# emreatilgan/P-Companion

Hardware: AMD Instinct MI355X
Metric: triplets/sec (Product2Vec pretrain step: gather+fwd+bwd+Adam) + P-Companion joint step under `joint` (higher is better)
Workload: dtype f32

## Files before the change

include/pcompanion_hip.h:

```cpp
#ifndef PCOMPANION_HIP_H
#define PCOMPANION_HIP_H

#include <stddef.h>
#include <stdint.h>

#ifdef __cplusplus
extern "C" {
#endif

#define PC_OK 0
#define PC_EINVAL (-1)
#define PC_ESHAPE (-2)
#define PC_EWORKSPACE (-3)
#define PC_EBATCHNORM (-4)
#define PC_ECOMM (-5)

#define PC_D 128
#define PC_H 256
#define PC_HEADS 4
#define PC_L 64
#define PC_MAX_SEG 4
#define PC_BN_SYNC_DOUBLES (PC_MAX_SEG * 2 * 256 + PC_MAX_SEG)

#define PC_ABI_VERSION 8
int pc_abi_version(void);
enum { PC_OPT_SIDE_QUEUE = 1, PC_OPT_SORTED_TABLE_GRADIENTS = 2, PC_OPT_BN_FINALIZE_SIDE = 3, PC_OPT_FUSED_LOSS = 4,
       PC_OPT_FUSED_OUT_CHAIN = 5, PC_OPT_BN_FINALIZE_RIDES = 6 };
int pc_set_option(int option, int value);
int pc_get_option(int option, int* value);
int pc_release_device_state(void);
enum {
    PC_FLAG_EXP_NO_MFMA = 1, PC_FLAG_EXP_NO_SPLIT = 2, PC_FLAG_EXP_NO_LDSREAD = 4, PC_FLAG_EXP_NO_DMA = 8,
    PC_FLAG_EXP_NO_SLAB = 16, PC_FLAG_EXP_STAGGER = 32, PC_FLAG_EXP_DMA_L2 = 64, PC_FLAG_NT_TIMING = 128,
    PC_FLAG_JOINT_TIMING = 256, PC_FLAG_CHAIN_TIMING = 512, PC_FLAG_EXP_NO_BARRIER = 1024, PC_FLAG_EXP_NO_VMWAIT = 2048
};
unsigned pc_build_flags(void);

typedef struct {
    float p;
    uint64_t seed, offset;
} pc_dropout;

typedef struct {
    float *w0, *b0, *gamma, *beta, *w3, *b3, *w5, *b5;
    float *in_proj_w, *in_proj_b, *out_proj_w, *out_proj_b;
    float *running_mean, *running_var;
    int64_t *num_batches_tracked;
    pc_dropout dropout;
    int dim;
} pc_p2v_tensors;

typedef struct {
    int nseg;
    int start[PC_MAX_SEG + 1];
    int count[PC_MAX_SEG];
    int weighted_row;
    float weight;
    const float *row_weight;
    int row_weight_start, row_weight_rows;
} pc_segments;
// ... 577 lines not shown
```

p_companion_amd/_lib.py:

```python
import ctypes
import os

_HERE = os.path.dirname(os.path.abspath(__file__))
LIB_PATH = os.path.join(_HERE, "libpcompanion_hip.so")
if os.environ.get("PC_DEV_LIB"):
    import sys as _sys
    LIB_PATH = os.path.abspath(os.environ["PC_DEV_LIB"])
    print(f"[p_companion_amd] PC_DEV_LIB: loading {LIB_PATH} instead of the in-tree library (developer A/B run)", file=_sys.stderr, flush=True)

c_f32p = ctypes.c_void_p
c_i32p = ctypes.c_void_p
PC_MAX_SEG = 4
D, H, HEADS, L = 128, 256, 4, 64

_ERR = {-1: "PC_EINVAL (null pointer / bad size)", -2: "PC_ESHAPE (unsupported dimension/alignment)",
        -3: "PC_EWORKSPACE (workspace too small)",
        -4: "PC_EBATCHNORM (a BatchNorm call group of one row in training mode)",
        -5: "PC_ECOMM (RCCL could not be loaded, or a communicator call failed)"}


class HipKernelError(RuntimeError):
    pass


# ... 20 lines not shown
class AttnSaved(ctypes.Structure):
    _fields_ = [(n, ctypes.c_void_p) for n in ("q", "qt", "probs", "c", "sp", "ctx")]


class JointTensors(ctypes.Structure):
    _fields_ = [(n, ctypes.c_void_p) for n in (
        "product_table", "enc_w", "enc_b", "dec_w", "dec_b", "typ_w", "typ_b", "itm_w", "itm_b",
        "query_types", "comp_types")] + [("dropout", Dropout)]


class JointSaved(ctypes.Structure):
    _fields_ = [(n, ctypes.c_void_p) for n in ("h", "c", "pi", "tp")]


_vp, _i, _sz, _f, _d, _u64, _i64 = (ctypes.c_void_p, ctypes.c_int, ctypes.c_size_t, ctypes.c_float,
                                    ctypes.c_double, ctypes.c_uint64, ctypes.c_int64)
_P = ctypes.POINTER

class AdamFused(ctypes.Structure):
    _fields_ = [("param", ctypes.c_void_p), ("grad", ctypes.c_void_p), ("exp_avg", ctypes.c_void_p), ("exp_avg_sq", ctypes.c_void_p),
                ("n", ctypes.c_size_t), ("step_count", ctypes.c_void_p), ("t", ctypes.c_int64),
                ("lr", ctypes.c_double), ("beta1", ctypes.c_double), ("beta2", ctypes.c_double), ("eps", ctypes.c_double)]


class RowWhere(ctypes.Structure):
    _fields_ = [(n, ctypes.c_void_p) for n in ("value", "lo", "hi", "flags", "need", "deny")]


PC_OPT_SIDE_QUEUE = 1
PC_OPT_FUSED_OUT_CHAIN = 5
PC_OPT_FUSED_LOSS = 4
PC_OPT_BN_FINALIZE_SIDE = 3
PC_OPT_BN_FINALIZE_RIDES = 6
PC_OPT_SORTED_TABLE_GRADIENTS = 2

SIGNATURES = {
    "pc_abi_version": (_i, []),
    "pc_build_flags": (ctypes.c_uint, []),
    "pc_set_option": (_i, [_i, _i]),
    "pc_get_option": (_i, [_i, ctypes.POINTER(ctypes.c_int)]),
    "pc_release_device_state": (_i, []),
    "pc_p2v_ffn_workspace_bytes": (_sz, [_i]),
    "pc_p2v_ffn_forward_train": (_i, [_P(P2VTensors), _vp, _vp, _i, _P(Segments), _i, _vp, _P(FfnSaved), _vp, _sz, _vp]),
    "pc_p2v_ffn_forward_eval": (_i, [_P(P2VTensors), _vp, _vp, _i, _vp, _vp, _sz, _vp]),
    "pc_p2v_ffn_backward": (_i, [_P(P2VTensors), _P(P2VTensors), _vp, _vp, _i, _P(Segments), _vp, _P(FfnSaved),
                                 _vp, _i, _vp, _sz, _vp]),
    "pc_p2v_attention_workspace_bytes": (_sz, [_i, _i]),
    "pc_p2v_attention_workspace_bytes_dim": (_sz, [_i, _i, _i]),
    "pc_p2v_attention_forward": (_i, [_P(P2VTensors), _vp, _vp, _i, _i, _vp, _P(AttnSaved), _vp, _sz, _vp]),
    "pc_p2v_attention_backward": (_i, [_P(P2VTensors), _P(P2VTensors), _vp, _vp, _i, _i, _vp, _P(AttnSaved), _vp,
                                       _vp, _i, _vp, _sz, _vp]),
    "pc_p2v_attention_forward_masked": (_i, [_P(P2VTensors), _vp, _vp, _vp, _i, _i, _vp, _P(AttnSaved), _vp, _sz, _vp]),
    "pc_p2v_attention_backward_masked": (_i, [_P(P2VTensors), _P(P2VTensors), _vp, _vp, _vp, _i, _i, _vp, _P(AttnSaved), _vp,
                                              _vp, _i, _vp, _sz, _vp]),
    "pc_p2v_train_step_compact_masked": (_i, [_P(P2VTensors), _P(P2VTensors), _vp, _vp, _vp, _vp, _vp, _i, _vp, _i, _i, _i, _f,
                                              _vp, _vp, _vp, _vp, _vp, _vp, _sz, _vp]),
    "pc_p2v_train_step_unique_masked": (_i, [_P(P2VTensors), _P(P2VTensors), _vp, _vp, _vp, _vp, _vp, _vp, _vp, _i, _i, _vp, _vp,
                                             _vp, _i, _i, _i, _f, _vp, _vp, _vp, _vp, _vp, _vp, _sz, _P(AdamFused), _vp]),
    "pc_p2v_export_workspace_bytes": (_sz, [_i, _i]),
    "pc_p2v_export_embeddings": (_i, [_P(P2VTensors), _vp, _i64, _vp, _vp, _vp, _vp, _i, _vp, _sz, _vp]),
    "pc_p2v_triplet_loss": (_i, [_vp, _vp, _vp, _i, _i, _f, _vp, _vp, _vp, _vp, _vp, _vp, _vp]),
    "pc_p2v_triplet_loss_dim": (_i, [_vp, _vp, _vp, _i, _i, _i, _f, _vp, _vp, _vp, _vp, _vp, _vp, _vp]),
    "pc_adam_step": (_i, [_vp, _vp, _vp, _vp, _sz, _vp, _vp, _d, _d, _d, _d, _vp]),
    "pc_adam_step_at": (_i, [_vp, _vp, _vp, _vp, _sz, _vp, _i64, _d, _d, _d, _d, _vp]),
    "pc_p2v_train_step_workspace_bytes": (_sz, [_i, _i, _i]),
    "pc_p2v_train_step_workspace_bytes_dim": (_sz, [_i, _i, _i, _i]),
# ... 214 lines not shown
```

p_companion_amd/csrc/common.h:

```cpp
#pragma once
#include <hip/hip_runtime.h>
#include <stdint.h>
#include "../../include/pcompanion_hip.h"

typedef float f32x16 __attribute__((ext_vector_type(16)));
typedef float f32x4 __attribute__((ext_vector_type(4)));

#define PC_WAVE 64

#define PC_HIP_TRY(expr)                          \
    do {                                          \
        hipError_t _e = (expr);                   \
        if (_e != hipSuccess) return (int)_e;     \
    } while (0)

#define PC_TRY(expr)                 \
    do {                             \
        int _r = (expr);             \
        if (_r != 0) return _r;      \
    } while (0)

extern thread_local int pc_tls_launch_err;
#define PC_LAUNCH(...)                                                           \
    do {                                                                         \
// ... 44 lines not shown
    for (int i = 0; i < PC_MAX_SEG; i++) {
        si.tile0[i] = t;
        int n = si.start[i + 1] - si.start[i];
        t += (n + tile_rows - 1) / tile_rows;
    }
    si.tile0[PC_MAX_SEG] = t;
    return si;
}

static inline int seg_valid(const pc_segments* s, int rows) {
    if (!s) return 1;
    if (s->nseg < 1 || s->nseg > PC_MAX_SEG || s->start[0] != 0 || s->start[s->nseg] != rows) return 0;
    for (int i = 0; i < s->nseg; i++)
        if (s->start[i + 1] < s->start[i] || s->count[i] < 0) return 0;
    if (s->weighted_row >= rows || (s->weighted_row >= 0 && s->weight < 0.f)) return 0;
    if (s->row_weight && (s->row_weight_start < 0 || s->row_weight_rows < 0 || s->row_weight_start + s->row_weight_rows > rows))
        return 0;
    return 1;
}

#ifdef __HIPCC__
__device__ __forceinline__ int seg_of_row(const SegInfo& si, int r) {
    int s = 0;
#pragma unroll
    for (int i = 1; i < PC_MAX_SEG; i++) s += (i < si.nseg && r >= si.start[i]) ? 1 : 0;
    return s;
}

__device__ __forceinline__ float row_multiplicity(const SegInfo& si, int r) {
#ifdef PC_EXP_NO_ROWMULT
    return 1.f;
#endif
    if (si.roww && (unsigned)(r - si.w0) < (unsigned)si.wn) return si.roww[r - si.w0];
    return r == si.wrow ? si.wmult : 1.f;
}

__device__ __forceinline__ int seg_of_tile(const SegInfo& si, int t) {
    int s = 0;
#pragma unroll
    for (int i = 1; i < PC_MAX_SEG; i++) s += (i < si.nseg && t >= si.tile0[i]) ? 1 : 0;
    return s;
}

__device__ __forceinline__ float fast_tanh(float x) {
    const float e = __builtin_amdgcn_exp2f(x * 2.8853900817779268f);
    return 1.0f - 2.0f * __builtin_amdgcn_rcpf(e + 1.0f);
}

__device__ __forceinline__ float wave_sum(float v) {
#pragma unroll
    for (int o = 32; o >= 1; o >>= 1) v += __shfl_xor(v, o, 64);
    return v;
}

__device__ __forceinline__ float group16_sum(float v) {
#pragma unroll
    for (int o = 8; o >= 1; o >>= 1) v += __shfl_xor(v, o, 64);
    return v;
}

__device__ __forceinline__ f32x16 mfma32(float a, float b, f32x16 c) {
    return __builtin_amdgcn_mfma_f32_32x32x2f32(a, b, c, 0, 0, 0);
}

typedef __bf16 bf16x8 __attribute__((ext_vector_type(8)));
struct Split3 { bf16x8 p0, p1, p2; };
// ... 364 lines not shown
int scatter_add_slab_blocks(int table_rows, int rows, int width);
int launch_scatter_add_slabs(const int32_t* idx, int rows, int width, int table_rows, const float* src, float* slabs,
                             hipStream_t st);

struct WsCarver {
    char* base; size_t total;
    explicit WsCarver(void* b) : base(static_cast<char*>(b)), total(0) {}
    void* bytes(size_t n) {
        void* p = base ? base + total : nullptr;
        total += (n + 255) & ~(size_t)255;
        return p;
    }
    float* floats(size_t n) { return static_cast<float*>(bytes(n * sizeof(float))); }
};

static inline void joint_fields(const pc_joint_tensors* t, float* (&out)[10]) {
    float* const f[10] = {t->itm_w, t->itm_b, t->typ_w, t->typ_b, t->dec_w, t->dec_b, t->enc_w, t->enc_b, t->comp_types, t->query_types};
    for (int i = 0; i < 10; i++) out[i] = f[i];
}
static inline bool joint_tensors_ok(const pc_joint_tensors* t, bool need_table) {
    if (!t || (need_table && !t->product_table)) return false;
    float* f[10];
    joint_fields(t, f);
    for (float* x : f)
        if (!x) return false;
    return true;
}

int pc_opt_sorted_tables();
int pc_opt_bn_finalize_side();
int pc_opt_bn_finalize_rides();
int pc_opt_fused_loss();
int pc_opt_fused_out_chain();
int triplet_loss_launch(const float* a, const float* p, const float* n, int batch, int k_neg, int dim, float margin,
                        float* loss, float* d_pos, float* d_neg, float* da, float* dp, float* dn, void* stream, int with_mean);
int launch_dropout(const float* x, size_t n, const pc_dropout& d, unsigned stream_id, float* y, hipStream_t st);
int launch_transpose(const float* in, int rows, int cols, float* out, hipStream_t st);
struct FfnCall {
    const pc_p2v_tensors *p = nullptr, *g = nullptr;
    const float* table = nullptr;
    const int32_t* idx = nullptr;
    int rows = 0;
    const pc_segments* seg = nullptr;
    const pc_ffn_saved* sv = nullptr;
    void* ws = nullptr; size_t ws_bytes = 0; void* stream = nullptr;
    double* local_sums = nullptr; const double* global_sums = nullptr;
    int update_running = 0; float* y = nullptr;
    const TransposeBatch* ride = nullptr;
    const float* dy = nullptr; float* dx = nullptr;
    int with_dx = 0, transposed = 0;
    int accumulate = 0;
    TnDefer* defer = nullptr;
};
int ffn_forward_part1(const FfnCall& c);
int ffn_forward_part2(const FfnCall& c);
int ffn_backward_part1(const FfnCall& c);
int ffn_backward_part2(const FfnCall& c);
int ffn_transposes(const pc_p2v_tensors* p, void* ws, int rows, int with_dx, TransposeBatch* tb);
int attention_transposes(const pc_p2v_tensors* p, void* ws, int B, int N, int key_rows, TransposeBatch* tb, float* zero_bk);
struct AttnCall {
    const pc_p2v_tensors* p = nullptr;
    const float *query = nullptr, *keys = nullptr;
    int B = 0, N = 0, key_rows = 0;
    const int32_t* slot_row = nullptr;
    const pc_attn_saved* sv = nullptr;
    void* ws = nullptr; size_t ws_bytes = 0; void* stream = nullptr;
// ... 29 lines not shown
```

p_companion_amd/csrc/gemm_tn.hip:

```cpp
#include <atomic>
#include <mutex>
#include <type_traits>
#include "common.h"
#include "bn_finalize.h"
#include "lds_dma.h"

#define TM 128
#define TK 32

__device__ __forceinline__ void tn_small_body(const TnArgs& a, int tiles_i, int nsplit, int rows_per_split, int bid) {
    __shared__ __attribute__((aligned(16))) float smem[2][2][TK * TM];

    const int tid = threadIdx.x, lane = tid & 63, w = tid >> 6, wo = w >> 1, wi = w & 1;
    const int split = bid % nsplit;
    const int tile = bid / nsplit;
    const int o0 = (tile / tiles_i) * TM, i0 = (tile % tiles_i) * TM;
    const int r_begin = split * rows_per_split;
    const int r_end = min(a.R, r_begin + rows_per_split);

    const int lrow = tid >> 5, lcol = (tid & 31) * 4;
    const bool zcol_ok = o0 + lcol < a.No, acol_ok = i0 + lcol < a.Ni;

    float4 rz[4], ra[4];
    float4 dbacc = make_float4(0.f, 0.f, 0.f, 0.f);
    int zseg = -1;
    float4 zmu, zis, zsc, zc1, zc2;
    auto gload = [&](int r0) {
#pragma unroll
        for (int p = 0; p < 4; p++) {
            const int r = r0 + lrow + 8 * p;
            const bool rv = r < r_end;
            if (a.z_onehot) {
                const int t = rv ? a.z_onehot[r] : -1, c = o0 + lcol;
                rz[p] = make_float4(t == c ? 1.f : 0.f, t == c + 1 ? 1.f : 0.f, t == c + 2 ? 1.f : 0.f, t == c + 3 ? 1.f : 0.f);
            } else {
                rz[p] = (rv && zcol_ok) ? *reinterpret_cast<const float4*>(a.Z + (size_t)r * a.ldz + o0 + lcol)
                                        : make_float4(0.f, 0.f, 0.f, 0.f);
            }
            if (a.zaux && rv && zcol_ok) {
                const int s = seg_of_row(a.seg, r);
                if (s != zseg) {
                    const size_t o = (size_t)s * a.No + o0 + lcol;
                    zmu = *reinterpret_cast<const float4*>(a.z_mean + o);
                    zis = *reinterpret_cast<const float4*>(a.z_invstd + o);
                    zsc = *reinterpret_cast<const float4*>(a.z_scale + o);
                    zc1 = *reinterpret_cast<const float4*>(a.z_c1 + o);
                    zc2 = *reinterpret_cast<const float4*>(a.z_c2 + o);
                    zseg = s;
                }
                const float4 h = *reinterpret_cast<const float4*>(a.zaux + (size_t)r * a.ldzaux + o0 + lcol);
                const float zm = row_multiplicity(a.seg, r);
                rz[p].x = zsc.x * (rz[p].x - zm * (zc1.x + (h.x - zmu.x) * zis.x * zc2.x));
                rz[p].y = zsc.y * (rz[p].y - zm * (zc1.y + (h.y - zmu.y) * zis.y * zc2.y));
                rz[p].z = zsc.z * (rz[p].z - zm * (zc1.z + (h.z - zmu.z) * zis.z * zc2.z));
                rz[p].w = zsc.w * (rz[p].w - zm * (zc1.w + (h.w - zmu.w) * zis.w * zc2.w));
            }
            int src = r;
            bool av = rv && acol_ok;
            if (av && a.gather) { src = a.gather[r]; av = src >= 0; }
            ra[p] = av ? *reinterpret_cast<const float4*>(a.A + (size_t)src * a.lda + i0 + lcol)
                       : make_float4(0.f, 0.f, 0.f, 0.f);
            if (a.prologue == NT_PRO_BNTANH && rv && acol_ok) {
                const int s = seg_of_row(a.seg, r);
                const float4 sc = *reinterpret_cast<const float4*>(a.pscale + (size_t)s * a.Ni + i0 + lcol);
                const float4 sh = *reinterpret_cast<const float4*>(a.pshift + (size_t)s * a.Ni + i0 + lcol);
                ra[p].x = fast_tanh(ra[p].x * sc.x + sh.x);
                ra[p].y = fast_tanh(ra[p].y * sc.y + sh.y);
                ra[p].z = fast_tanh(ra[p].z * sc.z + sh.z);
                ra[p].w = fast_tanh(ra[p].w * sc.w + sh.w);
            }
            dbacc.x += rz[p].x; dbacc.y += rz[p].y; dbacc.z += rz[p].z; dbacc.w += rz[p].w;
        }
    };
    auto lstore = [&](int buf) {
#pragma unroll
        for (int p = 0; p < 4; p++) {
            *reinterpret_cast<float4*>(&smem[buf][0][(lrow + 8 * p) * TM + lcol]) = rz[p];
            *reinterpret_cast<float4*>(&smem[buf][1][(lrow + 8 * p) * TM + lcol]) = ra[p];
        }
    };

    f32x16 acc[2][2];
#pragma unroll
    for (int i = 0; i < 2; i++)
#pragma unroll
        for (int j = 0; j < 2; j++)
#pragma unroll
            for (int r = 0; r < 16; r++) acc[i][j][r] = 0.f;
// ... 36 lines not shown
            for (int reg = 0; reg < 16; reg++) {
                const int o = o0 + wo * 64 + mt * 32 + (reg & 3) + 8 * (reg >> 2) + 4 * (lane >> 5);
                if (o < a.No && i < a.Ni) slab[(size_t)o * a.Ni + i] = acc[mt][nt][reg];
            }
        }
    if (a.db && i0 == 0) {
        float* red = &smem[0][0][0];
        *reinterpret_cast<float4*>(&red[lrow * TM + lcol]) = dbacc;
        __syncthreads();
        if (tid < TM && o0 + tid < a.No) {
            float s = 0.f;
#pragma unroll
            for (int g = 0; g < 8; g++) s += red[g * TM + tid];
            slab[(size_t)a.No * a.Ni + o0 + tid] = s;
        }
    }
}

__global__ __launch_bounds__(256, 2) void gemm_tn_kernel(TnArgs a, int tiles_i, int nsplit, int rows_per_split) {
    tn_small_body(a, tiles_i, nsplit, rows_per_split, blockIdx.x);
}

__global__ __launch_bounds__(256, 2) void gemm_tn_group_kernel(TnGroup g) {
    const int b = blockIdx.x;
    int j = 0;
#pragma unroll
    for (int i = 1; i < PC_TN_GROUP; i++) j += (i < g.n && b >= g.block0[i]) ? 1 : 0;
    tn_small_body(g.a[j], g.tiles_i[j], g.nsplit[j], g.rps[j], b - g.block0[j]);
}

__device__ __attribute__((aligned(64))) float pc_tn_zero_chunk[16];

struct TnNoRider {};
template <int WO, int WI, int TO, int TI, int TKC, int NST, bool APRO, bool ZPRO, bool RIDER = false>
__global__ __launch_bounds__(64 * WO * WI, WO * WI / 4) void gemm_tn8_kernel(TnArgs a, int nsplit, int rows_per_split, int halves,
                                                                             size_t slab_half_off,
                                                                             std::conditional_t<RIDER, TnRider, TnNoRider> rider) {
    constexpr int NWV = WO * WI, THREADS = 64 * NWV;
    constexpr int NO = WO * TO * 32, NI = WI * TI * 32;
    constexpr int ZRS = NO == 256 ? 260 : NO, ARS = NI == 256 ? 260 : NI;
    constexpr bool ZSW = NO == 128, ASW = NI == 128;
    static_assert((NO == 128 || NO == 256) && (NI == 128 || NI == 256), "image widths");
    constexpr int ZF = TKC * ZRS, AF = TKC * ARS;
    constexpr int STAGE = ZF * (ZPRO ? 2 : 1) + AF;
    constexpr int JZ = TKC * NO / 256 / NWV, JA = TKC * NI / 256 / NWV;
    static_assert((TKC * NO) % (256 * NWV) == 0 && (TKC * NI) % (256 * NWV) == 0, "images must split into whole wave instructions over the waves");
    constexpr int JALL = JZ * (ZPRO ? 2 : 1) + JA;
    __shared__ __attribute__((aligned(1024))) float smem[NST * STAGE];

    const int tid = threadIdx.x, lane = tid & 63;
    const int w = __builtin_amdgcn_readfirstlane(tid >> 6), wo = w % WO, wi = w / WO;
    const int half = halves == 2 ? ((int)blockIdx.x >> 3) & 1 : 0;
    const int split = halves == 2 ? (((int)blockIdx.x >> 4) << 3) + ((int)blockIdx.x & 7) : (int)blockIdx.x;
    if (halves == 2) {
        a.Z += half * (WO * TO * 32);
        a.slabs += half * slab_half_off;
        if (a.db) a.db += half * (WO * TO * 32);
    }
    const int r_begin = split * rows_per_split;
    const int r_end = min(a.R, r_begin + rows_per_split);
    const float* const zsrc0 = pc_tn_zero_chunk;
    const unsigned lds0 = (unsigned)(uintptr_t)(lptr_t)&smem[0];
    if constexpr (RIDER) {
        int rid = -1;
#pragma unroll
        for (int i = 0; i < PC_TN_RIDERS; i++) rid = (int)blockIdx.x == rider.block[i] ? i : rid;
        if (rid >= 0) {
            static_assert(sizeof(smem) >= sizeof(BnFinBwdScratch) && THREADS == FIN4_CG * FIN4_LANES, "a finalize workgroup");
            bn_finalize_bwd_body(rider.fin, rider.si, rid, (int)threadIdx.x, reinterpret_cast<BnFinBwdScratch*>(smem));
            return;
        }
    }

    int zr[JZ], zc[JZ], ar[JA], ac[JA];
    unsigned zd[JZ], ad[JA];
#pragma unroll
    for (int j = 0; j < JZ; j++) {
        const int g = w + NWV * j, f = g * 256 + lane * 4;
        zr[j] = f / NO; zc[j] = f % NO;
        if (ZSW && (zr[j] & 8)) zc[j] ^= 32;
        zd[j] = (NO == 256 ? g * ZRS : g * 256) * 4;
    }
#pragma unroll
    for (int j = 0; j < JA; j++) {
        const int g = w + NWV * j, f = g * 256 + lane * 4;
        ar[j] = f / NI; ac[j] = f % NI;
        if (ASW && (ar[j] & 8)) ac[j] ^= 32;
        ad[j] = (NI == 256 ? g * ARS : g * 256) * 4;
    }
    int gidx[JA];
    auto load_gather = [&](int r0) {
#pragma unroll
        for (int j = 0; j < JA; j++) {
            const int r = r0 + ar[j];
            gidx[j] = (a.gather && r < r_end) ? a.gather[r] : r;
        }
    };
    auto issue = [&](int st, int r0) {
        const unsigned base = lds0 + st * (STAGE * 4);
#pragma unroll
        for (int j = 0; j < JZ; j++) {
            const int r = r0 + zr[j];
            const bool v = r < r_end && zc[j] < a.No;
            dma16(v ? a.Z + (size_t)r * a.ldz + zc[j] : zsrc0, base + zd[j]);
            if (ZPRO) dma16(v ? a.zaux + (size_t)r * a.ldzaux + zc[j] : zsrc0, base + ZF * 4 + zd[j]);
        }
#pragma unroll
        for (int j = 0; j < JA; j++) {
            const int r = r0 + ar[j];
            const bool v = r < r_end && ac[j] < a.Ni && gidx[j] >= 0;
            dma16(v ? a.A + (size_t)gidx[j] * a.lda + ac[j] : zsrc0, base + (ZPRO ? 2 : 1) * ZF * 4 + ad[j]);
        }
    };

    constexpr int ZT = NO / 4, AT = NI / 4;
    const int zrow = tid / ZT, zcol = (tid % ZT) * 4, arow = tid / AT, acol = (tid % AT) * 4;
    int zseg = -1;
    float4 zmu, zis, zsc, zc1, zc2;
    auto transform = [&](float* stage, int r0) {
        if (ZPRO && zcol < a.No) {
            float* Zs = stage;
            const float* Hs = stage + ZF;
#pragma unroll
            for (int p = 0; p < TKC / (THREADS / ZT); p++) {
                const int rr = zrow + (THREADS / ZT) * p, r = r0 + rr;
                if (r < r_end) {
                    const int s = seg_of_row(a.seg, r);
                    if (s != zseg) {
                        const size_t o = (size_t)s * a.No + zcol;
                        zmu = *reinterpret_cast<const float4*>(a.z_mean + o);
                        zis = *reinterpret_cast<const float4*>(a.z_invstd + o);
                        zsc = *reinterpret_cast<const float4*>(a.z_scale + o);
                        zc1 = *reinterpret_cast<const float4*>(a.z_c1 + o);
                        zc2 = *reinterpret_cast<const float4*>(a.z_c2 + o);
                        zseg = s;
                    }
                    const int zp = rr * ZRS + ((ZSW && (rr & 8)) ? zcol ^ 32 : zcol);
                    float4 z = *reinterpret_cast<const float4*>(&Zs[zp]);
                    const float4 h = *reinterpret_cast<const float4*>(&Hs[zp]);
                    const float zm = row_multiplicity(a.seg, r);
                    z.x = zsc.x * (z.x - zm * (zc1.x + (h.x - zmu.x) * zis.x * zc2.x));
                    z.y = zsc.y * (z.y - zm * (zc1.y + (h.y - zmu.y) * zis.y * zc2.y));
                    z.z = zsc.z * (z.z - zm * (zc1.z + (h.z - zmu.z) * zis.z * zc2.z));
                    z.w = zsc.w * (z.w - zm * (zc1.w + (h.w - zmu.w) * zis.w * zc2.w));
                    *reinterpret_cast<float4*>(&Zs[zp]) = z;
                }
            }
        }
        if (APRO && acol < a.Ni) {
            float* As = stage + (ZPRO ? 2 : 1) * ZF;
            int aseg = -1;
            float4 asc, ash;
#pragma unroll
            for (int p = 0; p < TKC / (THREADS / AT); p++) {
                const int rr = arow + (THREADS / AT) * p, r = r0 + rr;
                if (r < r_end) {
                    const int s = seg_of_row(a.seg, r);
                    if (s != aseg) {
                        asc = *reinterpret_cast<const float4*>(a.pscale + (size_t)s * a.Ni + acol);
                        ash = *reinterpret_cast<const float4*>(a.pshift + (size_t)s * a.Ni + acol);
                        aseg = s;
                    }
                    const int ap = rr * ARS + ((ASW && (rr & 8)) ? acol ^ 32 : acol);
                    float4 x = *reinterpret_cast<const float4*>(&As[ap]);
                    x.x = fast_tanh(x.x * asc.x + ash.x);
                    x.y = fast_tanh(x.y * asc.y + ash.y);
                    x.z = fast_tanh(x.z * asc.z + ash.z);
                    x.w = fast_tanh(x.w * asc.w + ash.w);
                    *reinterpret_cast<float4*>(&As[ap]) = x;
                }
            }
        }
    };

    f32x16 acc[TO][TI];
    float zsum[TO];
#pragma unroll
    for (int i = 0; i < TO; i++) {
        zsum[i] = 0.f;
#pragma unroll
        for (int j = 0; j < TI; j++)
#pragma unroll
            for (int r = 0; r < 16; r++) acc[i][j][r] = 0.f;
    }

    const int nchunk = (r_end - r_begin + TKC - 1) / TKC;
#pragma unroll
    for (int i = 0; i < NST - 1; i++)
        if (i < nchunk) { load_gather(r_begin + i * TKC); issue(i, r_begin + i * TKC); }
    if (NST - 1 < nchunk) load_gather(r_begin + (NST - 1) * TKC);
    static_assert(TKC % 16 == 0, "chunks are whole k groups");
    const int fz = 8 * (lane >> 5) * ZRS, fa = 8 * (lane >> 5) * ARS;
    int zo[TO], xo[TI];
#pragma unroll
    for (int i = 0; i < TO; i++) zo[i] = (wo * (TO * 32) + 32 * i + (lane & 31)) ^ ((ZSW && lane >= 32) ? 32 : 0);
#pragma unroll
    for (int j = 0; j < TI; j++) xo[j] = (wi * (TI * 32) + 32 * j + (lane & 31)) ^ ((ASW && lane >= 32) ? 32 : 0);
    int cur = 0;
    for (int c = 0; c < nchunk; c++) {
#ifndef PC_EXP_NO_VMWAIT
        if (c + NST - 1 <= nchunk) { asm volatile("s_waitcnt vmcnt(%0)" ::"n"((NST - 2) * JALL) : "memory"); }
        else { asm volatile("s_waitcnt vmcnt(0)" ::: "memory"); }
#endif
#ifndef PC_EXP_NO_BARRIER
        __syncthreads();
#endif
#ifndef PC_EXP_NO_DMA
        if (c + NST - 1 < nchunk) {
            issue(cur == 0 ? NST - 1 : cur - 1, r_begin + (c + NST - 1) * TKC);
            if (c + NST < nchunk) load_gather(r_begin + (c + NST) * TKC);
        }
#endif
        float* stage = smem + cur * STAGE;
        if (APRO || ZPRO) { transform(stage, r_begin + c * TKC); lds_sync(); }
        const float* Zs = stage + fz;
        const float* As = stage + (ZPRO ? 2 : 1) * ZF + fa;
#pragma unroll
        for (int g = 0; g < TKC / 16; g++) {
#if defined(PC_EXP_NO_LDSREAD)
#define PC_TNV(PTR, OFF) __int_as_float(a.R + t)
#else
#define PC_TNV(PTR, OFF) (PTR)[OFF]
#endif
            Split3 sx[TI];
#pragma unroll
            for (int j = 0; j < TI; j++) {
                float v[8];
#pragma unroll
                for (int t = 0; t < 8; t++) v[t] = PC_TNV(As, (16 * g + t) * ARS + xo[j]);
                sx[j] = PC_SPLIT(make_float4(v[0], v[1], v[2], v[3]), make_float4(v[4], v[5], v[6], v[7]));
            }
#pragma unroll
            for (int i = 0; i < TO; i++) {
                float v[8];
#pragma unroll
                for (int t = 0; t < 8; t++) v[t] = PC_TNV(Zs, (16 * g + t) * ZRS + zo[i]);
                zsum[i] += ((v[0] + v[1]) + (v[2] + v[3])) + ((v[4] + v[5]) + (v[6] + v[7]));
                const Split3 sz = PC_SPLIT(make_float4(v[0], v[1], v[2], v[3]), make_float4(v[4], v[5], v[6], v[7]));
#define PC_TERM(PZ, PX) _Pragma("unroll") for (int j = 0; j < TI; j++) acc[i][j] = PC_MFMA(sz.PZ, sx[j].PX, acc[i][j]);
                PC_PRIO_MFMA(PC_PRIO_TN_COND, 1);
                PC_TERM(p2, p0) PC_TERM(p0, p2) PC_TERM(p1, p1) PC_TERM(p1, p0) PC_TERM(p0, p1) PC_TERM(p0, p0)
                PC_PRIO_MFMA(PC_PRIO_TN_COND, 0);
#undef PC_TERM
            }
        }
        cur = cur + 1 == NST ? 0 : cur + 1;
    }

    float* slab = a.slabs + (size_t)split * ((size_t)a.No * a.Ni + a.No);
// ... 133 lines not shown
    if (s < 1) s = 1;
    return (size_t)s * ((size_t)No * Ni + No);
}

static int tn_defer_push(TnDefer* d, const float* slabs, size_t slab_floats, int nsplit, int n_w, int n_b, float* dW,
                         float* db, int accumulate) {
    if (d->r.n >= PC_TN_RGROUP) return PC_EINVAL;
    const size_t used = (size_t)nsplit * ((size_t)n_w + n_b);
    if (used > slab_floats) return PC_EWORKSPACE;
    for (int k = 0; k < d->r.n; k++) {
        const float* lo = d->r.slabs[k];
        const float* hi = lo + (size_t)d->r.nsplit[k] * ((size_t)d->r.n_w[k] + d->r.n_b[k]);
        if (slabs < hi && lo < slabs + used) return PC_EINVAL;
    }
    const int k = d->r.n++;
    d->r.slabs[k] = slabs; d->r.nsplit[k] = nsplit; d->r.n_w[k] = n_w; d->r.n_b[k] = n_b; d->r.dW[k] = dW; d->r.db[k] = db;
    d->r.accumulate[k] = accumulate; d->r.block0[k] = d->rblocks;
    d->rblocks += ((n_w + (db ? n_b : 0)) / 4 * 8 + 255) / 256;
    return PC_OK;
}

int launch_gemm_tn(const TnArgs& a, hipStream_t st, TnDefer* defer) {
    if ((!a.Z && !a.z_onehot) || !a.A || !a.dW || !a.slabs || a.R <= 0 || a.No <= 0 || a.Ni <= 0) return PC_EINVAL;
    if (a.No % 4 || a.Ni % 4 || (a.Z && a.ldz % 4) || a.lda % 4 || a.lddw != a.Ni) return PC_ESHAPE;
    if (a.z_onehot && (a.zaux || tn_full_tile(a.R, a.No, a.Ni))) return PC_ESHAPE;
    if (((uintptr_t)a.dW & 15) || (a.db && ((uintptr_t)a.db & 15)) || ((uintptr_t)a.slabs & 15)) return PC_ESHAPE;
    int nsplit, rps;
    tn_plan(a.R, a.No, a.Ni, &nsplit, &rps);
    if ((size_t)nsplit * ((size_t)a.No * a.Ni + a.No) > a.slab_floats) return PC_EWORKSPACE;
    const int tiles_o = (a.No + TM - 1) / TM, tiles_i = (a.Ni + TM - 1) / TM;
    const bool apro = a.prologue == NT_PRO_BNTANH, zpro = a.zaux != nullptr;
    const int pb = pc_prof_begin(PC_KIND_GEMM_TN, 2.0 * a.R * (double)a.No * a.Ni, st);
    if (tn_full_tile(a.R, a.No, a.Ni) && !(apro && zpro)) {
#define TN8(WO, WI, TO, TI, TKC, NST)                                                                         \
    do {                                                                                                      \
        if (apro) PC_LAUNCH((gemm_tn8_kernel<WO, WI, TO, TI, TKC, NST, true, false>), dim3(nsplit), dim3(64 * WO * WI), 0, st, a, nsplit, rps, 1, (size_t)0, TnNoRider{});    \
        else if (zpro && a.Ni > 128) PC_LAUNCH((gemm_tn8_kernel<2, 4, 4, 2, 16, 3, false, true>), dim3(nsplit), dim3(512), 0, st, a, nsplit, rps, 1, (size_t)0, TnNoRider{});  \
        else if (zpro) PC_LAUNCH((gemm_tn8_kernel<4, 2, 2, 2, 16, 3, false, true>), dim3(nsplit), dim3(512), 0, st, a, nsplit, rps, 1, (size_t)0, TnNoRider{});  \
        else PC_LAUNCH((gemm_tn8_kernel<WO, WI, TO, TI, TKC, NST, false, false>), dim3(nsplit), dim3(64 * WO * WI), 0, st, a, nsplit, rps, 1, (size_t)0, TnNoRider{});        \
    } while (0)
        if (a.No > 128 && a.Ni > 128) TN8(2, 4, 4, 2, 16, 3);
        else if (a.No > 128) TN8(4, 2, 2, 2, 32, 2);
        else TN8(2, 4, 2, 2, 32, 2);
#undef TN8
    } else {
        PC_LAUNCH(gemm_tn_kernel, dim3(tiles_o * tiles_i * nsplit), dim3(256), 0, st, a, tiles_i, nsplit, rps);
    }
    pc_prof_end(pb, st);
    PC_TRY(pc_launch_status());
    const int n_w = a.No * a.Ni, n_b = a.No;
    const int threads = (n_w + (a.db ? n_b : 0)) / 4 * 8;
    if (defer) return tn_defer_push(defer, a.slabs, a.slab_floats, nsplit, n_w, n_b, a.dW, a.db, a.accumulate);
    PC_LAUNCH(tn_reduce_kernel, dim3((threads + 255) / 256), dim3(256), 0, st, a.slabs, nsplit, n_w, n_b,
                       a.dW, a.db, a.accumulate);
    return pc_launch_status();
}

int launch_gemm_tn_halves(const TnArgs& a, float* slabs0, float* slabs1, size_t slab_floats, hipStream_t st, TnDefer* defer,
                          const TnRider* rider) {
    if (!a.Z || !a.A || !a.dW || !slabs0 || !slabs1 || !defer || a.R <= 0) return PC_EINVAL;
    if (a.No != 256 || a.Ni != 256 || a.ldz % 4 || a.lda % 4 || a.lddw != a.Ni || a.prologue != NT_PRO_NONE || a.zaux || a.z_onehot || a.gather)
        return PC_ESHAPE;
    if (slabs1 < slabs0) return PC_EINVAL;
    const int nsplit = 128;
    int rps = (a.R + nsplit - 1) / nsplit;
    rps = (rps + 31) / 32 * 32;
    const int used = (a.R + rps - 1) / rps;
    const size_t per = (size_t)128 * a.Ni + 128;
    if ((size_t)nsplit * per > slab_floats) return PC_EWORKSPACE;
    TnArgs h = a;
    h.No = 128; h.slabs = slabs0; h.slab_floats = slab_floats;
    TnRider rd = {};
    int blocks = 2 * nsplit, nred = nsplit;
    if (rider && rider->n) {
        if (rider->n != PC_TN_RIDERS) return PC_EINVAL;
        rd = *rider;
        int k = 0;
        for (int b = 0; b < 2 * nsplit && k < rd.n; b++)
            if (((b >> 4) << 3) + (b & 7) >= used) rd.block[k++] = b;
        if (k == rd.n) nred = used;
        else {
            for (k = 0; k < rd.n; k++) rd.block[k] = blocks + k;
            blocks += rd.n;
        }
    }
    const int pb = pc_prof_begin(PC_KIND_GEMM_TN, 2.0 * a.R * (double)a.No * a.Ni, st);
    if (rd.n)
        PC_LAUNCH((gemm_tn8_kernel<2, 4, 2, 2, 32, 2, false, false, true>), dim3(blocks), dim3(512), 0, st, h, nsplit, rps, 2,
                  (size_t)(slabs1 - slabs0), rd);
    else
        PC_LAUNCH((gemm_tn8_kernel<2, 4, 2, 2, 32, 2, false, false>), dim3(blocks), dim3(512), 0, st, h, nsplit, rps, 2,
                  (size_t)(slabs1 - slabs0), TnNoRider{});
    pc_prof_end(pb, st);
    PC_TRY(pc_launch_status());
    PC_TRY(tn_defer_push(defer, slabs0, slab_floats, nred, 128 * a.Ni, 128, a.dW, a.db, a.accumulate));
    return tn_defer_push(defer, slabs1, slab_floats, nred, 128 * a.Ni, 128, a.dW + (size_t)128 * a.Ni, a.db ? a.db + 128 : nullptr,
                         a.accumulate);
}

namespace {
struct ForkSlot { int dev; hipStream_t main_st; int state; PcFork f; };
ForkSlot g_fork_slots[32];
std::mutex g_fork_mu;
std::atomic<int> g_opt_side_queue{1};
std::atomic<int> g_opt_sorted_tables{1};
std::atomic<int> g_opt_bn_finalize_side{0};
std::atomic<int> g_opt_bn_finalize_rides{1};
std::atomic<int> g_opt_fused_loss{1};
std::atomic<int> g_opt_fused_out_chain{1};
std::atomic<int>* opt_slot(int option) {
    switch (option) {
        case PC_OPT_SIDE_QUEUE: return &g_opt_side_queue;
        case PC_OPT_SORTED_TABLE_GRADIENTS: return &g_opt_sorted_tables;
        case PC_OPT_BN_FINALIZE_SIDE: return &g_opt_bn_finalize_side;
        case PC_OPT_FUSED_LOSS: return &g_opt_fused_loss;
        case PC_OPT_FUSED_OUT_CHAIN: return &g_opt_fused_out_chain;
        case PC_OPT_BN_FINALIZE_RIDES: return &g_opt_bn_finalize_rides;
        default: return nullptr;
    }
}
}
int pc_opt_sorted_tables() { return g_opt_sorted_tables.load(std::memory_order_relaxed); }
int pc_opt_bn_finalize_side() { return g_opt_bn_finalize_side.load(std::memory_order_relaxed); }
int pc_opt_bn_finalize_rides() { return g_opt_bn_finalize_rides.load(std::memory_order_relaxed); }
int pc_opt_fused_loss() { return g_opt_fused_loss.load(std::memory_order_relaxed); }
int pc_opt_fused_out_chain() { return g_opt_fused_out_chain.load(std::memory_order_relaxed); }

extern "C" int pc_set_option(int option, int value) {
    std::atomic<int>* o = opt_slot(option);
    if (!o || (value != 0 && value != 1)) return PC_EINVAL;
    o->store(value, std::memory_order_relaxed);
    return PC_OK;
}
extern "C" int pc_get_option(int option, int* value) {
    std::atomic<int>* o = opt_slot(option);
    if (!o || !value) return PC_EINVAL;
    *value = o->load(std::memory_order_relaxed);
    return PC_OK;
}
extern "C" int pc_release_device_state(void) {
    std::lock_guard<std::mutex> lock(g_fork_mu);
    int cur = 0, rc = PC_OK;
    const bool have_cur = hipGetDevice(&cur) == hipSuccess;
    for (ForkSlot& c : g_fork_slots) {
        if (c.state == 1) {
            if (hipSetDevice(c.dev) != hipSuccess) { rc = (int)hipErrorInvalidDevice; continue; }
            (void)hipStreamSynchronize(c.f.side);
            for (int i = 0; i < PC_FORK_EVENTS; i++) { (void)hipEventDestroy(c.f.fork[i]); (void)hipEventDestroy(c.f.join[i]); }
            (void)hipStreamDestroy(c.f.side);
        }
        c = ForkSlot{};
    }
    if (have_cur) (void)hipSetDevice(cur);
    return rc;
}

PcFork* pc_fork_get(hipStream_t main_st) {
    int dev = 0;
    if (!g_opt_side_queue.load(std::memory_order_relaxed) || hipGetDevice(&dev) != hipSuccess) return nullptr;
// ... 173 lines not shown
```

Baseline: 5.142 million.

## Load BN pre-activation H into registers instead of staging it in LDS for dW0 GEMM

For the TN weight-gradient GEMM with a BatchNorm-backward Z prologue (No<=128 path), the H tensor is now loaded directly into registers one chunk ahead via inline global loads, instead of being DMA'd into a second LDS image. This removes half of the Z-side LDS footprint and LDS traffic, and lets the default variant use TKC=32 with 2 stages. The transform now runs right after the barrier using register H, then prefetches the next chunk's H. An option (default off) restores the staged-LDS path. The risks are extra register pressure and exposed global-load latency.

```diff
diff --git a/include/pcompanion_hip.h b/include/pcompanion_hip.h
--- a/include/pcompanion_hip.h
+++ b/include/pcompanion_hip.h
@@ -25,7 +25,7 @@
 #define PC_ABI_VERSION 8
 int pc_abi_version(void);
 enum { PC_OPT_SIDE_QUEUE = 1, PC_OPT_SORTED_TABLE_GRADIENTS = 2, PC_OPT_BN_FINALIZE_SIDE = 3, PC_OPT_FUSED_LOSS = 4,
-       PC_OPT_FUSED_OUT_CHAIN = 5, PC_OPT_BN_FINALIZE_RIDES = 6 };
+       PC_OPT_FUSED_OUT_CHAIN = 5, PC_OPT_BN_FINALIZE_RIDES = 6, PC_OPT_DW0_STAGED_H = 7 };
 int pc_set_option(int option, int value);
 int pc_get_option(int option, int* value);
 int pc_release_device_state(void);
diff --git a/p_companion_amd/_lib.py b/p_companion_amd/_lib.py
--- a/p_companion_amd/_lib.py
+++ b/p_companion_amd/_lib.py
@@ -76,6 +76,7 @@
 PC_OPT_FUSED_LOSS = 4
 PC_OPT_BN_FINALIZE_SIDE = 3
 PC_OPT_BN_FINALIZE_RIDES = 6
+PC_OPT_DW0_STAGED_H = 7
 PC_OPT_SORTED_TABLE_GRADIENTS = 2
 
 SIGNATURES = {
diff --git a/p_companion_amd/csrc/common.h b/p_companion_amd/csrc/common.h
--- a/p_companion_amd/csrc/common.h
+++ b/p_companion_amd/csrc/common.h
@@ -100,6 +100,17 @@
     return 1.f;
 #endif
     if (si.roww && (unsigned)(r - si.w0) < (unsigned)si.wn) return si.roww[r - si.w0];
+    return r == si.wrow ? si.wmult : 1.f;
+}
+
+__device__ __forceinline__ const float* row_multiplicity_src(const SegInfo& si, int r, const float* none) {
+    return (si.roww && (unsigned)(r - si.w0) < (unsigned)si.wn) ? si.roww + (r - si.w0) : none;
+}
+__device__ __forceinline__ float row_multiplicity_from(const SegInfo& si, int r, float listed) {
+#ifdef PC_EXP_NO_ROWMULT
+    return 1.f;
+#endif
+    if (si.roww && (unsigned)(r - si.w0) < (unsigned)si.wn) return listed;
     return r == si.wrow ? si.wmult : 1.f;
 }
 
@@ -530,6 +541,7 @@
 int pc_opt_bn_finalize_rides();
 int pc_opt_fused_loss();
 int pc_opt_fused_out_chain();
+int pc_opt_dw0_staged_h();
 int triplet_loss_launch(const float* a, const float* p, const float* n, int batch, int k_neg, int dim, float margin,
                         float* loss, float* d_pos, float* d_neg, float* da, float* dp, float* dn, void* stream, int with_mean);
 int launch_dropout(const float* x, size_t n, const pc_dropout& d, unsigned stream_id, float* y, hipStream_t st);
diff --git a/p_companion_amd/csrc/gemm_tn.hip b/p_companion_amd/csrc/gemm_tn.hip
--- a/p_companion_amd/csrc/gemm_tn.hip
+++ b/p_companion_amd/csrc/gemm_tn.hip
@@ -7,6 +7,15 @@
 
 #define TM 128
 #define TK 32
+
+__device__ __forceinline__ float4 bn_bwd_z4(float4 z, const float4& h, float zm, const float4& mu, const float4& is,
+                                            const float4& sc, const float4& c1, const float4& c2) {
+    z.x = sc.x * (z.x - zm * (c1.x + (h.x - mu.x) * is.x * c2.x));
+    z.y = sc.y * (z.y - zm * (c1.y + (h.y - mu.y) * is.y * c2.y));
+    z.z = sc.z * (z.z - zm * (c1.z + (h.z - mu.z) * is.z * c2.z));
+    z.w = sc.w * (z.w - zm * (c1.w + (h.w - mu.w) * is.w * c2.w));
+    return z;
+}
 
 __device__ __forceinline__ void tn_small_body(const TnArgs& a, int tiles_i, int nsplit, int rows_per_split, int bid) {
     __shared__ __attribute__((aligned(16))) float smem[2][2][TK * TM];
@@ -50,10 +59,7 @@
                 }
                 const float4 h = *reinterpret_cast<const float4*>(a.zaux + (size_t)r * a.ldzaux + o0 + lcol);
                 const float zm = row_multiplicity(a.seg, r);
-                rz[p].x = zsc.x * (rz[p].x - zm * (zc1.x + (h.x - zmu.x) * zis.x * zc2.x));
-                rz[p].y = zsc.y * (rz[p].y - zm * (zc1.y + (h.y - zmu.y) * zis.y * zc2.y));
-                rz[p].z = zsc.z * (rz[p].z - zm * (zc1.z + (h.z - zmu.z) * zis.z * zc2.z));
-                rz[p].w = zsc.w * (rz[p].w - zm * (zc1.w + (h.w - zmu.w) * zis.w * zc2.w));
+                rz[p] = bn_bwd_z4(rz[p], h, zm, zmu, zis, zsc, zc1, zc2);
             }
             int src = r;
             bool av = rv && acol_ok;
@@ -156,20 +162,31 @@
 __device__ __attribute__((aligned(64))) float pc_tn_zero_chunk[16];
 
 struct TnNoRider {};
+typedef float tn_v4f __attribute__((ext_vector_type(4)));
+__device__ __forceinline__ void tn_tie_h(tn_v4f (&h)[4]) { asm volatile("" : "+v"(h[0]), "+v"(h[1]), "+v"(h[2]), "+v"(h[3])::"memory"); }
+__device__ __forceinline__ void tn_tie_h(tn_v4f (&h)[2]) { asm volatile("" : "+v"(h[0]), "+v"(h[1])::"memory"); }
+#ifdef PC_EXP_DW0_REGH_16X3
+#define PC_TN_REGH_ALL 1
+#else
+#define PC_TN_REGH_ALL 0
+#endif
 template <int WO, int WI, int TO, int TI, int TKC, int NST, bool APRO, bool ZPRO, bool RIDER = false>
 __global__ __launch_bounds__(64 * WO * WI, WO * WI / 4) void gemm_tn8_kernel(TnArgs a, int nsplit, int rows_per_split, int halves,
                                                                              size_t slab_half_off,
                                                                              std::conditional_t<RIDER, TnRider, TnNoRider> rider) {
+    constexpr bool REGH = ZPRO && (TKC == 32 || (PC_TN_REGH_ALL && WO == 4));
+    static_assert(!REGH || (!APRO && !RIDER), "register H is a form of the ZPRO loader");
     constexpr int NWV = WO * WI, THREADS = 64 * NWV;
     constexpr int NO = WO * TO * 32, NI = WI * TI * 32;
     constexpr int ZRS = NO == 256 ? 260 : NO, ARS = NI == 256 ? 260 : NI;
     constexpr bool ZSW = NO == 128, ASW = NI == 128;
     static_assert((NO == 128 || NO == 256) && (NI == 128 || NI == 256), "image widths");
     constexpr int ZF = TKC * ZRS, AF = TKC * ARS;
-    constexpr int STAGE = ZF * (ZPRO ? 2 : 1) + AF;
+    constexpr int ZIMG = (ZPRO && !REGH) ? 2 : 1;
+    constexpr int STAGE = ZF * ZIMG + AF;
     constexpr int JZ = TKC * NO / 256 / NWV, JA = TKC * NI / 256 / NWV;
     static_assert((TKC * NO) % (256 * NWV) == 0 && (TKC * NI) % (256 * NWV) == 0, "images must split into whole wave instructions over the waves");
-    constexpr int JALL = JZ * (ZPRO ? 2 : 1) + JA;
+    constexpr int JALL = JZ * ZIMG + JA;
     __shared__ __attribute__((aligned(1024))) float smem[NST * STAGE];
 
     const int tid = threadIdx.x, lane = tid & 63;
@@ -227,13 +244,13 @@
             const int r = r0 + zr[j];
             const bool v = r < r_end && zc[j] < a.No;
             dma16(v ? a.Z + (size_t)r * a.ldz + zc[j] : zsrc0, base + zd[j]);
-            if (ZPRO) dma16(v ? a.zaux + (size_t)r * a.ldzaux + zc[j] : zsrc0, base + ZF * 4 + zd[j]);
+            if (ZIMG == 2) dma16(v ? a.zaux + (size_t)r * a.ldzaux + zc[j] : zsrc0, base + ZF * 4 + zd[j]);
         }
 #pragma unroll
         for (int j = 0; j < JA; j++) {
             const int r = r0 + ar[j];
             const bool v = r < r_end && ac[j] < a.Ni && gidx[j] >= 0;
-            dma16(v ? a.A + (size_t)gidx[j] * a.lda + ac[j] : zsrc0, base + (ZPRO ? 2 : 1) * ZF * 4 + ad[j]);
+            dma16(v ? a.A + (size_t)gidx[j] * a.lda + ac[j] : zsrc0, base + ZIMG * ZF * 4 + ad[j]);
         }
     };
 
@@ -241,12 +258,25 @@
     const int zrow = tid / ZT, zcol = (tid % ZT) * 4, arow = tid / AT, acol = (tid % AT) * 4;
     int zseg = -1;
     float4 zmu, zis, zsc, zc1, zc2;
+    constexpr int HP = TKC / (THREADS / ZT);
+    [[maybe_unused]] tn_v4f hreg[HP];
+    [[maybe_unused]] float hmult[HP];
+    [[maybe_unused]] auto load_h = [&](int r0) {
+#pragma unroll
+        for (int p = 0; p < HP; p++) {
+            const int r = r0 + zrow + (THREADS / ZT) * p;
+            const bool v = r < r_end && zcol < a.No;
+            const float* src = v ? a.zaux + (size_t)r * a.ldzaux + zcol : zsrc0;
+            asm volatile("global_load_dwordx4 %0, %1, off" : "=v"(hreg[p]) : "v"(src) : "memory");
+            hmult[p] = *(v ? row_multiplicity_src(a.seg, r, zsrc0) : zsrc0);
+        }
+    };
     auto transform = [&](float* stage, int r0) {
         if (ZPRO && zcol < a.No) {
             float* Zs = stage;
             const float* Hs = stage + ZF;
 #pragma unroll
-            for (int p = 0; p < TKC / (THREADS / ZT); p++) {
+            for (int p = 0; p < HP; p++) {
                 const int rr = zrow + (THREADS / ZT) * p, r = r0 + rr;
                 if (r < r_end) {
                     const int s = seg_of_row(a.seg, r);
@@ -260,19 +290,19 @@
                         zseg = s;
                     }
                     const int zp = rr * ZRS + ((ZSW && (rr & 8)) ? zcol ^ 32 : zcol);
-                    float4 z = *reinterpret_cast<const float4*>(&Zs[zp]);
-                    const float4 h = *reinterpret_cast<const float4*>(&Hs[zp]);
-                    const float zm = row_multiplicity(a.seg, r);
-                    z.x = zsc.x * (z.x - zm * (zc1.x + (h.x - zmu.x) * zis.x * zc2.x));
-                    z.y = zsc.y * (z.y - zm * (zc1.y + (h.y - zmu.y) * zis.y * zc2.y));
-                    z.z = zsc.z * (z.z - zm * (zc1.z + (h.z - zmu.z) * zis.z * zc2.z));
-                    z.w = zsc.w * (z.w - zm * (zc1.w + (h.w - zmu.w) * zis.w * zc2.w));
-                    *reinterpret_cast<float4*>(&Zs[zp]) = z;
+                    const float4 z = *reinterpret_cast<const float4*>(&Zs[zp]);
+                    float4 h;
+                    if constexpr (REGH) h = make_float4(hreg[p].x, hreg[p].y, hreg[p].z, hreg[p].w);
+                    else h = *reinterpret_cast<const float4*>(&Hs[zp]);
+                    float zm;
+                    if constexpr (REGH) zm = row_multiplicity_from(a.seg, r, hmult[p]);
+                    else zm = row_multiplicity(a.seg, r);
+                    *reinterpret_cast<float4*>(&Zs[zp]) = bn_bwd_z4(z, h, zm, zmu, zis, zsc, zc1, zc2);
                 }
             }
         }
         if (APRO && acol < a.Ni) {
-            float* As = stage + (ZPRO ? 2 : 1) * ZF;
+            float* As = stage + ZIMG * ZF;
             int aseg = -1;
             float4 asc, ash;
 #pragma unroll
@@ -313,6 +343,13 @@
     for (int i = 0; i < NST - 1; i++)
         if (i < nchunk) { load_gather(r_begin + i * TKC); issue(i, r_begin + i * TKC); }
     if (NST - 1 < nchunk) load_gather(r_begin + (NST - 1) * TKC);
+    if constexpr (REGH) {
+        if (nchunk > 0) {
+            load_h(r_begin);
+            asm volatile("s_waitcnt vmcnt(0)" ::: "memory");
+            tn_tie_h(hreg);
+        }
+    }
     static_assert(TKC % 16 == 0, "chunks are whole k groups");
     const int fz = 8 * (lane >> 5) * ZRS, fa = 8 * (lane >> 5) * ARS;
     int zo[TO], xo[TI];
@@ -325,10 +362,19 @@
 #ifndef PC_EXP_NO_VMWAIT
         if (c + NST - 1 <= nchunk) { asm volatile("s_waitcnt vmcnt(%0)" ::"n"((NST - 2) * JALL) : "memory"); }
         else { asm volatile("s_waitcnt vmcnt(0)" ::: "memory"); }
+        if constexpr (REGH) {
+            tn_tie_h(hreg);
+#pragma unroll
+            for (int j = 0; j < JA; j++) asm volatile("" : "+v"(gidx[j]));
+        }
 #endif
 #ifndef PC_EXP_NO_BARRIER
         __syncthreads();
 #endif
+        if constexpr (REGH) {
+            transform(smem + cur * STAGE, r_begin + c * TKC);
+            if (c + 1 < nchunk) load_h(r_begin + (c + 1) * TKC);
+        }
 #ifndef PC_EXP_NO_DMA
         if (c + NST - 1 < nchunk) {
             issue(cur == 0 ? NST - 1 : cur - 1, r_begin + (c + NST - 1) * TKC);
@@ -336,9 +382,10 @@
         }
 #endif
         float* stage = smem + cur * STAGE;
-        if (APRO || ZPRO) { transform(stage, r_begin + c * TKC); lds_sync(); }
+        if constexpr (REGH) lds_sync();
+        else if (APRO || ZPRO) { transform(stage, r_begin + c * TKC); lds_sync(); }
         const float* Zs = stage + fz;
-        const float* As = stage + (ZPRO ? 2 : 1) * ZF + fa;
+        const float* As = stage + ZIMG * ZF + fa;
 #pragma unroll
         for (int g = 0; g < TKC / 16; g++) {
 #if defined(PC_EXP_NO_LDSREAD)
@@ -538,10 +585,16 @@
     const bool apro = a.prologue == NT_PRO_BNTANH, zpro = a.zaux != nullptr;
     const int pb = pc_prof_begin(PC_KIND_GEMM_TN, 2.0 * a.R * (double)a.No * a.Ni, st);
     if (tn_full_tile(a.R, a.No, a.Ni) && !(apro && zpro)) {
+#if PC_TN_REGH_ALL
+#define TN8_REGH gemm_tn8_kernel<4, 2, 2, 2, 16, 3, false, true>
+#else
+#define TN8_REGH gemm_tn8_kernel<4, 2, 2, 2, 32, 2, false, true>
+#endif
 #define TN8(WO, WI, TO, TI, TKC, NST)                                                                         \
     do {                                                                                                      \
         if (apro) PC_LAUNCH((gemm_tn8_kernel<WO, WI, TO, TI, TKC, NST, true, false>), dim3(nsplit), dim3(64 * WO * WI), 0, st, a, nsplit, rps, 1, (size_t)0, TnNoRider{});    \
         else if (zpro && a.Ni > 128) PC_LAUNCH((gemm_tn8_kernel<2, 4, 4, 2, 16, 3, false, true>), dim3(nsplit), dim3(512), 0, st, a, nsplit, rps, 1, (size_t)0, TnNoRider{});  \
+        else if (zpro && !pc_opt_dw0_staged_h()) PC_LAUNCH((TN8_REGH), dim3(nsplit), dim3(512), 0, st, a, nsplit, rps, 1, (size_t)0, TnNoRider{});  \
         else if (zpro) PC_LAUNCH((gemm_tn8_kernel<4, 2, 2, 2, 16, 3, false, true>), dim3(nsplit), dim3(512), 0, st, a, nsplit, rps, 1, (size_t)0, TnNoRider{});  \
         else PC_LAUNCH((gemm_tn8_kernel<WO, WI, TO, TI, TKC, NST, false, false>), dim3(nsplit), dim3(64 * WO * WI), 0, st, a, nsplit, rps, 1, (size_t)0, TnNoRider{});        \
     } while (0)
@@ -549,6 +602,7 @@
         else if (a.No > 128) TN8(4, 2, 2, 2, 32, 2);
         else TN8(2, 4, 2, 2, 32, 2);
 #undef TN8
+#undef TN8_REGH
     } else {
         PC_LAUNCH(gemm_tn_kernel, dim3(tiles_o * tiles_i * nsplit), dim3(256), 0, st, a, tiles_i, nsplit, rps);
     }
@@ -614,8 +668,10 @@
 std::atomic<int> g_opt_bn_finalize_rides{1};
 std::atomic<int> g_opt_fused_loss{1};
 std::atomic<int> g_opt_fused_out_chain{1};
+std::atomic<int> g_opt_dw0_staged_h{0};
 std::atomic<int>* opt_slot(int option) {
     switch (option) {
+        case PC_OPT_DW0_STAGED_H: return &g_opt_dw0_staged_h;
         case PC_OPT_SIDE_QUEUE: return &g_opt_side_queue;
         case PC_OPT_SORTED_TABLE_GRADIENTS: return &g_opt_sorted_tables;
         case PC_OPT_BN_FINALIZE_SIDE: return &g_opt_bn_finalize_side;
@@ -631,6 +687,7 @@
 int pc_opt_bn_finalize_rides() { return g_opt_bn_finalize_rides.load(std::memory_order_relaxed); }
 int pc_opt_fused_loss() { return g_opt_fused_loss.load(std::memory_order_relaxed); }
 int pc_opt_fused_out_chain() { return g_opt_fused_out_chain.load(std::memory_order_relaxed); }
+int pc_opt_dw0_staged_h() { return g_opt_dw0_staged_h.load(std::memory_order_relaxed); }
 
 extern "C" int pc_set_option(int option, int value) {
     std::atomic<int>* o = opt_slot(option);
```

Result: faster. 5.248 million, median of 6 (+2.1%).
